# clearmatics/libff

Measured on AMD Instinct MI355X. Metric: G1 MSM throughput (scalar-muls/sec), higher is better.
Workload: dtype u32

## Files before the change

### libff_amd/build.py

```python
import concurrent.futures
import os
import shutil
import subprocess
import sys

HERE = os.path.dirname(os.path.abspath(__file__))
CSRC = os.path.join(HERE, "csrc")
OBJ = os.path.join(CSRC, "build")
INCLUDE = os.path.join(os.path.dirname(HERE), "include")
SO_PATH = os.path.join(HERE, "libamdmsm.so")

GROUPS = ["alt_bn128_g1", "alt_bn128_g2", "bls12_377_g1", "bls12_377_g2", "bw6_761_g1", "bw6_761_g2",
          "bls12_381_g1", "bls12_381_g2", "mnt4_g1", "mnt4_g2", "mnt6_g1"]
GROUP_FLAGS = {g: ["-DAMDMSM_HOT_INLINE=1", "-DAMDMSM_BENCH_BOTH=1"] for g in GROUPS}
GROUP_FLAGS["alt_bn128_g1"] = GROUP_FLAGS["alt_bn128_g1"] + ["-DAMDMSM_OVERLAP_OK=1"]
for _g in ("bls12_377_g2", "bls12_381_g2", "bw6_761_g1", "bw6_761_g2"):
    GROUP_FLAGS[_g] = GROUP_FLAGS[_g] + ["-DAMDMSM_ACC_WAVES=2"]
for _g in ("alt_bn128_g1", "bls12_377_g1", "bls12_381_g1"):
    GROUP_FLAGS[_g] = GROUP_FLAGS[_g] + ["-DAMDMSM_COLD_INLINE=1"]
for _g in ("bls12_377_g2", "bls12_381_g2", "alt_bn128_g2"):
    GROUP_FLAGS[_g] = GROUP_FLAGS[_g] + ["-DAMDMSM_ACC_SPLIT=1"]
GROUP_FLAGS["alt_bn128_g2"] = GROUP_FLAGS["alt_bn128_g2"] + ["-DAMDMSM_ACC_WAVES=3"]
for _g in ("bls12_377_g1", "bls12_381_g1"):
    GROUP_FLAGS[_g] = GROUP_FLAGS[_g] + ["-DAMDMSM_ACC_WAVES=3"]
for _g, _w in (("alt_bn128_g1", 3), ("bls12_377_g1", 2), ("bls12_381_g1", 2), ("bw6_761_g1", 2), ("bw6_761_g2", 2),
               ("alt_bn128_g2", 3), ("bls12_377_g2", 2), ("bls12_381_g2", 2)):
    GROUP_FLAGS[_g] = [f for f in GROUP_FLAGS[_g] if not f.startswith("-DAMDMSM_ACC_WAVES=")] + ["-DAMDMSM_ACC_RR=1", f"-DAMDMSM_ACC_WAVES={_w}"]
for _g in ("mnt4_g1", "mnt6_g1"):
    GROUP_FLAGS[_g] = GROUP_FLAGS[_g] + ["-DAMDMSM_COLD_INLINE=1", "-DAMDMSM_ACC_WAVES=3"]
GROUP_FLAGS["mnt4_g2"] = GROUP_FLAGS["mnt4_g2"] + ["-DAMDMSM_ACC_WAVES=2"]
ARCH = "gfx950"
COMMON = ["-O3", "-std=c++17", "-fPIC", f"--offload-arch={ARCH}", "-I" + INCLUDE, "-I" + CSRC,
          "-Wno-unused-result"]
DEVICE_DEPS = ["msm_group.hip", "rr.cuh", "rr_chain.inc", "fp.cuh", "fp2.cuh", "fp2h.cuh", "ec.cuh", "wide.cuh", "wide28.cuh", "mac_chain.inc", "curve_params.h", "group_vtable.h", os.path.join(HERE, "build.py")]
HOST_DEPS = ["engine.cpp", "ffi.cpp", "engine_internal.h", "group_vtable.h", os.path.join(INCLUDE, "amdmsm.h"),
             os.path.join(INCLUDE, "libff_amd_ffi.h")]


def hipcc():
    exe = shutil.which("hipcc") or "/opt/rocm/bin/hipcc"
    if not os.path.exists(exe):
        raise RuntimeError("hipcc not found: the amdmsm engine is HIP-only and cannot be built without ROCm")
    return exe


def _newer(target, deps):
    if not os.path.exists(target):
        return True
# ... 55 lines not shown
```

### libff_amd/csrc/engine.cpp

```cpp
#include "../../include/amdmsm.h"
#include "engine_internal.h"
#include "group_vtable.h"

#include <hip/hip_runtime.h>

#include <fcntl.h>
#include <sys/stat.h>
#include <unistd.h>

#include <algorithm>
#include <cmath>
#include <cstdio>
#include <cstdlib>
#include <cstring>
#include <mutex>
#include <string>
#include <thread>
#include <vector>

using namespace amdmsm;

constexpr int MAX_SLOTS = 4;
constexpr int MAX_GROUPS = 4;
struct ws_slot {
// ... 251 lines not shown
    p.off_plast = off;
    off = align_up(off + Wt * p.T * zz_bytes, 256);
    p.off_cont = off;
    off = align_up(off + Wt * p.T * 4, 256);
    p.G = G_req > 0 ? std::min(std::min(G_req, MAX_GROUPS), p.W) : 1;
    p.off_queue = off;
    p.queue_stride = align_up(fixup_queue_words((size_t)((p.W + p.G - 1) / p.G) * (size_t)batch * p.T) * 4, 256);
    off = off + p.queue_stride * p.G;
    p.off_partial = off;
    off = align_up(off + (size_t)MAX_GROUPS * xyz_bytes, 256);
    p.off_coarse = off;
    off = align_up(off + Wt * 1025 * 4, 256);
    p.off_big = off;
    p.big_stride = p.c <= 22 ? align_up(std::max(sort_geometry(n, p.c, p.W).big_words, big_words_min) * 4, 256) : 256;
    off += p.big_stride * (size_t)batch;
    p.off_cursor = off;
    off = align_up(off + Wt * 1024 * 4, 256);
    p.off_tmp_payload = off;
    off = align_up(off + Wt * p.list_stride * 4, 256);
    p.off_tmp_key = off;
    off = align_up(off + Wt * p.list_stride * 4, 256);
    p.off_endo = off;
    p.endo_stride = glv ? align_up((n / 2) * (size_t)vt->el_words * 2 * 4, 256) : 0;
    off += p.endo_stride * (size_t)batch;
    {
        static const int rc_env = getenv("AMDMSM_ROWCOL") ? atoi(getenv("AMDMSM_ROWCOL")) : 1;
        static const int rc_min_c = getenv("AMDMSM_ROWCOL_MIN_C") ? atoi(getenv("AMDMSM_ROWCOL_MIN_C")) : 10;
        static const int qr_env = getenv("AMDMSM_ROWCOL_QROW") ? atoi(getenv("AMDMSM_ROWCOL_QROW")) : 0;
        static const int qc_env = getenv("AMDMSM_ROWCOL_QCOL") ? atoi(getenv("AMDMSM_ROWCOL_QCOL")) : 0;
        p.rowcol = rc_env != 0 && p.c >= rc_min_c;
        const int h = p.c / 2;
        const size_t C = (size_t)1 << h, R = p.B >> h;
        const bool one_wave = vt->fq_words >= 24 || vt->el_words > vt->fq_words;
        const size_t lane_budget = one_wave ? 70000 : 140000;
        uint32_t q = 4;
        while (q < 64 && Wt * p.B * red_lanes * 2 / q > lane_budget) q <<= 1;
        p.q_row = qr_env > 0 ? (uint32_t)qr_env : q;
        p.q_col = qc_env > 0 ? (uint32_t)qc_env : q;
        p.rc_points = R + 1 + C;
        p.off_rc = off;
        off = align_up(off + Wt * p.rc_points * xyz_bytes, 256);
        p.off_planes = off;
        off = align_up(off + Wt * p.c * xyz_bytes, 256);
        p.off_winsum = off;
        off = align_up(off + Wt * xyz_bytes, 256);
    }
    p.total = off;
    return AMDMSM_OK;
}

int ensure_ws(amdmsm_ctx *ctx, ws_slot &sl, size_t bytes) {
    if (sl.ws_bytes >= bytes) return AMDMSM_OK;
    if (sl.ws) {
        HIP_TRY(ctx, hipDeviceSynchronize());
        HIP_TRY(ctx, hipFree(sl.ws));
        sl.ws = nullptr;
        sl.ws_bytes = 0;
    }
    const size_t want = bytes + bytes / 8;
    HIP_TRY(ctx, hipMalloc(&sl.ws, want));
    sl.ws_bytes = want;
    return AMDMSM_OK;
}

constexpr uint64_t TIMING_RING = 64;
void record(amdmsm_ctx *ctx, ws_slot &sl, int idx, hipStream_t st) {
    (void)sl;
// ... 2012 lines not shown
```

### libff_amd/csrc/group_vtable.h

```cpp
#pragma once
#include <hip/hip_runtime_api.h>
#include <stddef.h>
#include <stdint.h>
#include <stdlib.h>

namespace amdmsm {

enum out_form : int {
    OUT_JACOBIAN = 0,
    OUT_LIBFF = 1,
    OUT_AFFINE = 2,
};

struct sort_geom {
    int hb;
    int fb;
    uint32_t chunk_cap;
    uint32_t big_thresh;
    uint32_t big_cap;
    size_t big_words;
};
inline sort_geom sort_geometry(size_t n, int c, int W) {
    sort_geom g;
    static const int hb_env = getenv("AMDMSM_SORT_HB") ? atoi(getenv("AMDMSM_SORT_HB")) : 0;
    g.hb = c / 2 < 10 ? c / 2 : 10;
    if (c == 16 && n >= ((size_t)3 << 18) && n < ((size_t)3 << 19)) g.hb = 7;
    if (hb_env > 0) g.hb = hb_env;
    if (g.hb > c - 1) g.hb = c - 1;
    if (g.hb < 1) g.hb = 1;
    if (c - 1 - g.hb > 11) g.hb = c - 1 - 11;
    g.fb = c - 1 - g.hb;
    g.chunk_cap = 1024;
    static const uint32_t chunk_max = getenv("AMDMSM_SORT_CHUNK_MAX") ? (uint32_t)atoi(getenv("AMDMSM_SORT_CHUNK_MAX")) : 16384u;
    while (g.chunk_cap < chunk_max && g.chunk_cap < 2 * (n >> g.hb)) g.chunk_cap <<= 1;
    g.big_thresh = 16 * g.chunk_cap;
    g.big_cap = (uint32_t)((size_t)W * n / g.big_thresh + 1);
    g.big_words = 4 + (size_t)g.big_cap * 4 + ((size_t)g.big_cap << g.fb);
    return g;
}

#ifdef __HIPCC__
#define AMDMSM_HD __host__ __device__
#else
#define AMDMSM_HD
#endif
AMDMSM_HD inline size_t fixup_queue_cap_long(size_t lanes) { return lanes / 32 + 2; }
AMDMSM_HD inline size_t fixup_queue_cap_mid(size_t lanes) { return lanes / 3 + 2; }
inline size_t fixup_queue_words(size_t lanes) { return 2 + 2 * (fixup_queue_cap_long(lanes) + fixup_queue_cap_mid(lanes)); }

struct group_vtable {
    int curve, group;
    int fr_words;
    int el_words;
    int fq_words;
    int fr_bits;
    int projective;
    int reduce_fold;
    int bucket_words;
    const uint32_t* fr_one_mont;
    int glv_bound_log2_x1000;
    int prime_order;
    const uint32_t* glv_lambda;
    void (*endo_points)(hipStream_t, const uint32_t* bases_affine, size_t n, uint32_t* out);
    void (*glv_digits)(hipStream_t, const uint32_t* scalars, size_t n, int mont, int c, int W, int32_t* out);

    void (*import_bases)(hipStream_t, const uint32_t* src, size_t stride_words, int form_special,
                         size_t n, uint32_t* dst_affine);
    void (*precompute_table)(hipStream_t, const uint32_t* bases_affine, size_t n, int c, int D, uint32_t* tmp,
                             uint32_t* table);
    void (*count)(hipStream_t, const uint32_t* scalars, size_t n, int mont, int c, int W, uint32_t* counts);
    void (*scatter)(hipStream_t, const uint32_t* scalars, size_t n, int mont, int c, int W, uint32_t* cursor,
                    uint32_t* lists, size_t list_stride);
    void (*scalar_stats)(hipStream_t, const uint32_t* scalars, size_t n, int mont, uint32_t* stats);
    void (*sort)(hipStream_t, const uint32_t* scalars, size_t n, int mont, int c, int W, uint32_t* coarse,
                 uint32_t* cursor, int32_t* digits, uint32_t* tmp_payload, uint32_t* tmp_key, uint32_t* ends,
                 uint32_t* lists, size_t stride, uint32_t* big, int mode, hipEvent_t after_coarse);
    void (*accumulate)(hipStream_t, const uint32_t* ends, const uint32_t* lists, size_t list_stride,
                       const uint32_t* bases_affine, uint32_t* buckets, uint32_t* part_first, uint32_t* part_last,
                       uint32_t* cont_bucket, int W, uint32_t B, uint32_t S, uint32_t T, const uint32_t* endo_points,
                       size_t n_real, int overlap);
    size_t (*accumulate_resident_lanes)(int overlap);
    int accumulate_overlap_ok;
    void (*accumulate_fixup)(hipStream_t, const uint32_t* ends, uint32_t* buckets, uint32_t* part_first,
                             const uint32_t* part_last, const uint32_t* cont_bucket, uint32_t* queue, int W,
                             uint32_t B, uint32_t S, uint32_t T);
    void (*reduce_segments)(hipStream_t, const uint32_t* buckets, int W, uint32_t B, uint32_t L, uint32_t* out);
    void (*sum_butterfly)(hipStream_t, const uint32_t* in, int W, uint32_t M, uint32_t* out);
    void (*sum_block)(hipStream_t, const uint32_t* in, int W, uint32_t M, uint32_t* out);
    void (*reduce_rowcol)(hipStream_t, const uint32_t* buckets, int W, uint32_t B, int c, uint32_t q_row, uint32_t q_col,
                          uint32_t* rc, uint32_t* planes, uint32_t* out);
    void (*horner)(hipStream_t, const uint32_t* window_sums, int W, int c, int form, const uint32_t* init,
                   uint32_t* out);
    void (*horner_batch)(hipStream_t, const uint32_t* window_sums, int k, int W, int c, int form, uint32_t* const* outs);
    void (*sum_points)(hipStream_t, const uint32_t* pts, int k, int form, uint32_t* out);
    void (*gen_bases_seq)(hipStream_t, unsigned long long first, size_t n, uint32_t* dst_affine);
    void (*export_affine)(hipStream_t, const uint32_t* src_affine, size_t n, uint32_t* dst_xyz);

    void (*ffi_decode_points)(hipStream_t, const uint32_t* src_be, size_t n, uint32_t* dst_affine, uint32_t* status);
    void (*ffi_decode_scalars)(hipStream_t, const uint32_t* src_be, size_t n, uint32_t* dst_plain, uint32_t* status);
    void (*ffi_encode_point)(hipStream_t, const uint32_t* src_xyz_affine, uint32_t* dst_be);

    void (*disk_decode)(hipStream_t, const uint32_t* src, size_t n, uint32_t* dst_affine);
    void (*disk_decode_compressed)(hipStream_t, const uint32_t* src, size_t n, uint32_t* dst_affine, uint32_t* status);
    void (*fixed_base_exp)(hipStream_t, const uint32_t* g_xyz, int scalar_size, int window, const uint32_t* scalars,
                           size_t n, int mont, const uint32_t* coeff, int form, uint32_t* gouter, uint32_t* table,
                           uint32_t* table_aff, int build_table, uint32_t* out);

    void (*field_op)(hipStream_t, int op, const uint32_t* a, const uint32_t* b, uint32_t* out, size_t n);
    void (*group_op)(hipStream_t, int op, const uint32_t* a, const uint32_t* b, uint32_t* out, size_t n, int form);
    void (*digits)(hipStream_t, const uint32_t* scalars, size_t n, int mont, int c, int W, int32_t* out);
    void (*mul_bench)(hipStream_t, uint32_t* inout, size_t nthreads, int iters, int inline_variant);
    void (*madd_bench)(hipStream_t, const uint32_t* pts_affine, uint32_t* out_xyz, size_t nthreads, int iters,
                       int inline_variant);

    int has_endomorphism;
    int coeff_a_nonzero;

    void (*sort_sel)(hipStream_t, const uint32_t* shared, size_t shared_n, const uint32_t* index, size_t offset,
                     uint32_t* flag, size_t n, int mont, int c, int W, uint32_t* coarse, uint32_t* cursor, int32_t* digits,
                     uint32_t* tmp_payload, uint32_t* tmp_key, uint32_t* ends, uint32_t* lists, size_t stride, uint32_t* big,
                     int mode);
    void (*gather_scalars)(hipStream_t, const uint32_t* shared, size_t shared_n, const uint32_t* index, size_t offset,
                           uint32_t* flag, size_t n, uint32_t* out);
// ... 16 lines not shown
```

### libff_amd/csrc/msm_group.hip

```cpp
#include "curve_params.h"
#include "ec.cuh"
#include "fp2h.cuh"
#include "group_vtable.h"
#include "wide.cuh"
#include "wide28.cuh"
#include "rr.cuh"

#include <algorithm>
#include <cstdio>
#include <vector>
#include <type_traits>

#ifndef AMDMSM_GROUP
#error "compile with -DAMDMSM_GROUP=<group traits> -DAMDMSM_VT=<vtable getter name>"
#endif

namespace amdmsm {
template <bool I>
struct ec_coeff_a<Fp<AMDMSM_GROUP::fq, I>> {
    static constexpr int value = AMDMSM_GROUP::DEG == 1 ? AMDMSM_GROUP::COEFF_A : 0;
};
template <int NR, bool I>
struct ec_coeff_a<Fp2<AMDMSM_GROUP::fq, NR, I>> {
    static constexpr int value = AMDMSM_GROUP::DEG == 2 ? AMDMSM_GROUP::COEFF_A : 0;
};
namespace {

using GP = AMDMSM_GROUP;
using FQ = typename GP::fq;
using FR = typename GP::fr;
static_assert(GP::COEFF_A == 0 || (!GP::HAS_ENDO && GP::SUBGROUP_CHECK == 0 && GP::LIBFF_PROJECTIVE),
              "a != 0 is implemented for the MNT groups: no endomorphism, no subgroup test, projective records");
#if AMDMSM_ACC_RR || AMDMSM_ACC_SPLIT
static_assert(GP::COEFF_A == 0, "the reduced-radix and lane-pair accumulation loops are written for a = 0");
#endif

#ifndef AMDMSM_HOT_INLINE
#define AMDMSM_HOT_INLINE 0
#endif
#ifndef AMDMSM_BENCH_BOTH
#define AMDMSM_BENCH_BOTH 0
#endif
#ifndef AMDMSM_ACC_LAZY
#define AMDMSM_ACC_LAZY 1
#endif
#ifndef AMDMSM_ACC_WAVES
#define AMDMSM_ACC_WAVES 1
#endif
#ifndef AMDMSM_OVERLAP_OK
#define AMDMSM_OVERLAP_OK 0
#endif
#ifndef AMDMSM_TAIL_WAVES
#define AMDMSM_TAIL_WAVES 1
#endif
template <int DEG, bool I> struct coord_sel;
template <bool I> struct coord_sel<1, I> { using type = Fp<FQ, I>; };
template <bool I> struct coord_sel<2, I> { using type = Fp2<FQ, GP::NR_SMALL == 0 ? -1 : GP::NR_SMALL, I>; };
#ifndef AMDMSM_COLD_INLINE
#define AMDMSM_COLD_INLINE 0
#endif
using E = typename coord_sel<GP::DEG, (AMDMSM_COLD_INLINE != 0)>::type;
using EH = typename coord_sel<GP::DEG, (AMDMSM_HOT_INLINE != 0)>::type;
using EI = typename coord_sel<GP::DEG, true>::type;
#ifndef AMDMSM_ACC_SPLIT
#define AMDMSM_ACC_SPLIT 0
#endif
template <int DEG> struct split_sel { using type = EH; static constexpr int LANES = 1; };
#if AMDMSM_ACC_SPLIT
template <> struct split_sel<2> { using type = Fp2H<FQ, (GP::NR_SMALL == 0 ? -1 : GP::NR_SMALL)>; static constexpr int LANES = 2; };
#endif
using EA = typename split_sel<GP::DEG>::type;
constexpr int ACC_LANES = split_sel<GP::DEG>::LANES;
using ER = typename std::conditional<(ACC_LANES == 2), EA, E>::type;
constexpr int RED_LANES = ACC_LANES;
constexpr uint32_t RED_FOLD = 64u / RED_LANES;
#if AMDMSM_ACC_RR
static_assert(GP::DEG == 1 || AMDMSM_ACC_SPLIT, "reduced-radix Fq2 accumulation works on lane pairs");
template <int DEG> struct rr_el_sel { using type = Rr<FQ>; };
template <> struct rr_el_sel<2> { using type = Rr2H<FQ, (GP::NR_SMALL == 0 ? -1 : GP::NR_SMALL)>; };
using ERR = typename rr_el_sel<GP::DEG>::type;
#endif

constexpr int EW = FQ::N * GP::DEG;
constexpr int AFFW = 2 * EW;
constexpr int XYZW = 3 * EW;
constexpr int ZZW = 4 * EW;
#ifndef AMDMSM_ACC_RR
// ... 608 lines not shown
                                                        uint32_t perchunk_words, uint32_t* __restrict__ big,
                                                        uint32_t* __restrict__ ends, uint32_t* __restrict__ lists) {
    extern __shared__ __attribute__((aligned(16))) uint32_t smem[];
    __shared__ uint32_t tmp[NT / 64 + 1];
    const uint32_t nbin = 1u << hb;
    const int fb = c - 1 - hb;
    const uint32_t nfine = 1u << fb, fmask = nfine - 1u;
    uint32_t* fstart = smem;
    uint32_t* chist = fstart + nfine;
    uint32_t* cstart = chist + nfine;
    uint32_t* ccur = cstart + nfine;
    uint32_t* st_payload = ccur + nfine;
    unsigned short* st_fine = reinterpret_cast<unsigned short*>(st_payload + chunk_cap);
    const uint32_t bin = blockIdx.x, w = blockIdx.y;
    const uint32_t* cs = coarse + (size_t)w * (nbin + 1);
    const uint32_t b0 = cs[bin], m = cs[bin + 1] - b0;
    const sort_key_t* key = tmp_key + (size_t)w * stride + b0;
    const uint32_t* pay = tmp_payload + (size_t)w * stride + b0;
    uint32_t* out = lists + (size_t)w * stride + b0;
    uint32_t* e = ends + (((size_t)w << (c - 1)) + ((size_t)bin << fb));
    if (m > big_thresh) {
        for (uint32_t j = threadIdx.x; j < nfine; j += NT) e[j] = 0;
        if (threadIdx.x == 0) {
            const uint32_t tiles = (m + SORT_TILE - 1) / SORT_TILE;
            const uint32_t slot = atomicAdd(&big[0], 1u);
            uint32_t* rec = big + 4 + 4 * (size_t)slot;
            rec[0] = w;
            rec[1] = bin;
            rec[2] = atomicAdd(&big[1], tiles);
            rec[3] = tiles;
        }
        return;
    }
    if (m <= chunk_cap) {
        constexpr int PER = 16;
        uint32_t fk[PER], rk[PER];
        for (uint32_t j = threadIdx.x; j < nfine; j += NT) chist[j] = 0;
        __syncthreads();
#pragma unroll
        for (int q = 0; q < PER; ++q) {
            const uint32_t k = threadIdx.x + (uint32_t)q * NT;
            fk[q] = k < m ? (uint32_t)(key[k] & fmask) : 0u;
            rk[q] = k < m ? atomicAdd(&chist[fk[q]], 1u) : 0u;
        }
        __syncthreads();
        block_exclusive_scan<NT>(chist, fstart, nfine, tmp);
        for (uint32_t j = threadIdx.x; j < nfine; j += NT) e[j] = b0 + fstart[j] + chist[j];
#pragma unroll
        for (int q = 0; q < PER; ++q) {
            const uint32_t k = threadIdx.x + (uint32_t)q * NT;
            if (k < m) st_payload[fstart[fk[q]] + rk[q]] = pay[k];
        }
        __syncthreads();
        for (uint32_t k = threadIdx.x; k < m; k += NT) out[k] = st_payload[k];
        return;
    }
    const uint32_t nch = (m + chunk_cap - 1) / chunk_cap;
    const bool single = false;
    uint32_t* ch = reinterpret_cast<uint32_t*>(st_fine + chunk_cap);
    const bool split_hist = !single && (size_t)nch * nfine <= perchunk_words;
    if (split_hist) {
        int sh = 0;
        while ((1u << sh) < chunk_cap) ++sh;
        for (uint32_t j = threadIdx.x; j < nch * nfine; j += NT) ch[j] = 0;
        __syncthreads();
        for (uint32_t k = threadIdx.x; k < m; k += NT) atomicAdd(&ch[(k >> sh) * nfine + (key[k] & fmask)], 1u);
        __syncthreads();
        for (uint32_t j = threadIdx.x; j < nfine; j += NT) {
            uint32_t t = 0;
            for (uint32_t q = 0; q < nch; ++q) t += ch[q * nfine + j];
            chist[j] = t;
        }
    } else {
        for (uint32_t j = threadIdx.x; j < nfine; j += NT) chist[j] = 0;
        __syncthreads();
        for (uint32_t k = threadIdx.x; k < m; k += NT) atomicAdd(&chist[key[k] & fmask], 1u);
    }
    __syncthreads();
    block_exclusive_scan<NT>(chist, fstart, nfine, tmp);
    for (uint32_t j = threadIdx.x; j < nfine; j += NT) e[j] = b0 + fstart[j] + chist[j];
    __syncthreads();
    uint32_t cidx = 0;
    for (uint32_t c0 = 0; c0 < m; c0 += chunk_cap, ++cidx) {
        const uint32_t cm = (m - c0 < chunk_cap) ? m - c0 : chunk_cap;
        const uint32_t* hist_c = split_hist ? ch + cidx * nfine : chist;
        if (single) {
            for (uint32_t j = threadIdx.x; j < nfine; j += NT) cstart[j] = ccur[j] = fstart[j];
        } else {
            if (!split_hist) {
                for (uint32_t j = threadIdx.x; j < nfine; j += NT) chist[j] = 0;
                __syncthreads();
                for (uint32_t k = threadIdx.x; k < cm; k += NT) atomicAdd(&chist[key[c0 + k] & fmask], 1u);
                __syncthreads();
            }
            block_exclusive_scan<NT>(hist_c, cstart, nfine, tmp);
            for (uint32_t j = threadIdx.x; j < nfine; j += NT) ccur[j] = cstart[j];
        }
        __syncthreads();
        for (uint32_t k = threadIdx.x; k < cm; k += NT) {
            const uint32_t f = key[c0 + k] & fmask;
            const uint32_t r = atomicAdd(&ccur[f], 1u);
            st_payload[r] = pay[c0 + k];
            st_fine[r] = (unsigned short)f;
        }
        __syncthreads();
        for (uint32_t k = threadIdx.x; k < cm; k += NT) {
            const uint32_t f = st_fine[k];
            out[fstart[f] + (k - cstart[f])] = st_payload[k];
        }
        __syncthreads();
        for (uint32_t j = threadIdx.x; j < nfine; j += NT) fstart[j] += hist_c[j];
        __syncthreads();
    }
}

struct big_tile {
    uint32_t rec, w, bin, k0, cm;
};
AMDMSM_DEV bool big_find_tile(const uint32_t* __restrict__ big, const uint32_t* __restrict__ coarse, uint32_t nbin,
                              uint32_t tile, uint32_t* sh, big_tile& bt, uint32_t& b0) {
    const uint32_t nbig = big[0];
    __syncthreads();
    for (uint32_t r = threadIdx.x; r < nbig; r += SORT_TPB) {
        const uint32_t* rec = big + 4 + 4 * (size_t)r;
        if (tile >= rec[2] && tile < rec[2] + rec[3]) sh[0] = r;
    }
    __syncthreads();
    bt.rec = sh[0];
    const uint32_t* rec = big + 4 + 4 * (size_t)bt.rec;
    bt.w = rec[0];
// ... 247 lines not shown
        for (int j = 0; j < 4; ++j) {
            const int i = 4 * k + j;
            int32_t& dst = i < RRL ? re_limb(p.x, i) : (i < 2 * RRL ? re_limb(p.y, i - RRL) : (i < 3 * RRL ? re_limb(p.zz, i - 2 * RRL) : re_limb(p.zzz, i - 3 * RRL)));
            dst = (int32_t)w[j];
            if (i >= 2 * RRL && i < 3 * RRL) any |= w[j];
        }
    }
    inf = re_all<ERR>(any == 0);
    const bool rho = re_limb(p.zz, 0) < 0;
    if (rho) re_limb(p.zz, 0) &= 0x7fffffff;
    else xyzz_rec_to_rho(p);
}
AMDMSM_DEV void rec_sum_store(uint32_t* q, const rec_sum& s) {
    uint4* q4 = reinterpret_cast<uint4*>(q + (GP::DEG == 2 && (threadIdx.x & 1u) ? 4 * RRL : 0));
    uint32_t w[4 * RRL];
    const uint32_t keep = s.inf ? 0u : 0xffffffffu;
#pragma unroll
    for (int i = 0; i < RRL; ++i) {
        w[i] = (uint32_t)re_limb(s.a.x, i) & keep;
        w[RRL + i] = (uint32_t)re_limb(s.a.y, i) & keep;
        w[2 * RRL + i] = (uint32_t)re_limb(s.a.zz, i) & keep;
        w[3 * RRL + i] = (uint32_t)re_limb(s.a.zzz, i) & keep;
    }
    w[2 * RRL] |= 0x80000000u & keep;
#pragma unroll
    for (int i = 0; i < RRL; ++i) q4[i] = make_uint4(w[4 * i], w[4 * i + 1], w[4 * i + 2], w[4 * i + 3]);
}
AMDMSM_DEV void rec_sum_add(rec_sum& s, const uint32_t* q) {
    XyzzRr<ERR> b;
    bool b_inf;
    rec_load_rho(b, b_inf, q);
    xyzz_add_rho(s.a, s.inf, b, b_inf);
}
AMDMSM_DEV void rec_sum_fold(rec_sum& s, uint32_t G) {
    for (uint32_t off = 1; off < G; off <<= 1) {
        XyzzRr<ERR> o;
        const int m = (int)(off * RED_LANES);
#pragma unroll
        for (int i = 0; i < RRL; ++i) {
            re_limb(o.x, i) = __shfl_xor(re_limb(s.a.x, i), m, 64);
            re_limb(o.y, i) = __shfl_xor(re_limb(s.a.y, i), m, 64);
            re_limb(o.zz, i) = __shfl_xor(re_limb(s.a.zz, i), m, 64);
            re_limb(o.zzz, i) = __shfl_xor(re_limb(s.a.zzz, i), m, 64);
        }
        const bool o_inf = __shfl_xor(s.inf ? 1 : 0, m, 64) != 0;
        xyzz_add_rho(s.a, s.inf, o, o_inf);
    }
}
AMDMSM_DEV void rec_sum_get(Xyzz<ER>& out, const rec_sum& s) {
    if (s.inf) {
        xyzz_set_inf(out);
        return;
    }
    rr_export_component<FQ, 0>(lane_words(out.x), re_comp(s.a.x));
    rr_export_component<FQ, 0>(lane_words(out.y), re_comp(s.a.y));
    rr_export_component<FQ, 0>(lane_words(out.zz), re_comp(s.a.zz));
    rr_export_component<FQ, 0>(lane_words(out.zzz), re_comp(s.a.zzz));
}
#else
struct rec_sum {
    Xyzz<ER> a;
};
AMDMSM_DEV void rec_sum_init(rec_sum& s) { xyzz_set_inf(s.a); }
AMDMSM_DEV void rec_sum_add(rec_sum& s, const uint32_t* q) {
    Xyzz<ER> x;
    load_xyzz_rec(x, q);
    xyzz_add(s.a, s.a, x);
}
AMDMSM_DEV void rec_sum_get(Xyzz<ER>& out, const rec_sum& s) { out = s.a; }
AMDMSM_DEV void rec_sum_store(uint32_t* q, const rec_sum& s) { store_xyzz_rec(q, s.a); }
AMDMSM_DEV void wave_group_sum_r(Jac<ER>& p, uint32_t G);
AMDMSM_DEV void rec_sum_fold(rec_sum& s, uint32_t G) {
    Jac<ER> j;
    xyzz_to_jac(j, s.a);
    wave_group_sum_r(j, G);
    jac_to_xyzz(s.a, j);
}
#endif

AMDMSM_DEV uint32_t bucket_of_entry(const uint32_t* __restrict__ e, uint32_t B, uint32_t k) {
    uint32_t l = 0, r = B - 1;
    while (l < r) {
        const uint32_t m = (l + r) >> 1;
        if (e[m] > k) r = m; else l = m + 1;
    }
    return l;
}

__global__ void __launch_bounds__(TPB, AMDMSM_ACC_WAVES) k_accumulate(const uint32_t* __restrict__ ends, const uint32_t* __restrict__ lists,
                                                    size_t list_stride, const uint32_t* __restrict__ bases,
                                                    uint32_t* __restrict__ buckets, uint32_t* __restrict__ part_first,
                                                    uint32_t* __restrict__ part_last, uint32_t* __restrict__ cont_bucket,
                                                    int W, uint32_t B, uint32_t S, uint32_t T,
                                                    const uint32_t* __restrict__ endo_pts, uint32_t n_real, int sync_waves
#ifdef AMDMSM_ACC_TRACE
                                                    , unsigned long long* __restrict__ trace
#endif
                                                    ) {
#ifdef AMDMSM_ACC_TRACE
    const unsigned long long t_start = __builtin_amdgcn_s_memrealtime();
    struct trace_end {
// ... 394 lines not shown
            o[EW + env.j] = Y1;
            o[2 * EW + env.j] = Z1;
        }
    }
}
__global__ void __launch_bounds__(SUMW_THREADS) k_sum_block_wide(const uint32_t* __restrict__ in, int W, uint32_t M,
                                                                 uint32_t* __restrict__ out) {
    __shared__ uint32_t buf[2][SUMW_SLOTS * XYZW];
    __builtin_amdgcn_s_setprio(3);
    const size_t w = blockIdx.x;
    const uint32_t i = threadIdx.x / RED_LANES, wave = threadIdx.x >> 6;
    constexpr uint32_t NWAVES = SUMW_THREADS / 64;
    Jac<ER> p;
    if (i < M) load_jac(p, in + (w * M + i) * XYZW); else jac_set_inf(p);
    wave_group_sum_r(p, 4);
    if ((i & 3u) == 0) store_jac(buf[0] + (size_t)(i >> 2) * XYZW, p);
    __syncthreads();
    const WideEnv<FQ> env = wide_env<FQ>();
    uint32_t K = (M + 3) / 4;
    int cur = 0;
    while (K > 1) {
        const uint32_t pairs = K / 2;
        for (uint32_t q = wave; q < pairs; q += NWAVES) {
            const uint32_t* a = buf[cur] + (size_t)(2 * q) * XYZW;
            sum_wide_add(env, a, a + XYZW, buf[cur ^ 1] + (size_t)q * XYZW);
        }
        __syncthreads();
        cur ^= 1;
        K = pairs;
    }
    for (uint32_t t = threadIdx.x; t < (uint32_t)XYZW; t += SUMW_THREADS) out[w * XYZW + t] = buf[cur][t];
}

__global__ void __launch_bounds__(64, AMDMSM_TAIL_WAVES) k_bucket_sums(const uint32_t* __restrict__ buckets, int W, uint32_t B, int h,
                                                    uint32_t q_row, uint32_t q_col, uint32_t row_blocks,
                                                    uint32_t* __restrict__ out) {
    __builtin_amdgcn_s_setprio(3);
    const bool col = blockIdx.x >= row_blocks;
    const size_t t = ((size_t)(blockIdx.x - (col ? row_blocks : 0u)) * 64 + threadIdx.x) / RED_LANES;
    const uint32_t C = 1u << h, R = B >> h;
    const uint32_t q = col ? q_col : q_row, len = col ? R : C;
    const uint32_t g = len / q;
    const uint32_t nout = col ? C : R + 1;
    const size_t per_w = (size_t)nout * g;
    const size_t w = t / per_w;
    const uint32_t rem = (uint32_t)(t % per_w), o = rem / g, j = rem % g;
    const bool valid = w < (size_t)W;
    rec_sum sum;
    rec_sum_init(sum);
    if (valid) {
        const uint32_t* bk = buckets + w * (size_t)B * ZZS;
        for (uint32_t i = 0; i < q; ++i) {
            const uint32_t idx = j * q + i;
            const uint64_t b1 = col ? (uint64_t)idx * C + o : (uint64_t)o * C + idx;
            if (b1 >= 1 && b1 <= B) rec_sum_add(sum, bk + (size_t)(b1 - 1) * ZZS);
        }
    }
    rec_sum_fold(sum, g);
    Xyzz<ER> xa;
    rec_sum_get(xa, sum);
    Jac<ER> p;
    xyzz_to_jac(p, xa);
    if (valid && j == 0) store_jac(out + (w * (size_t)(R + 1 + C) + (col ? R + 1 + o : o)) * XYZW, p);
}

__global__ void __launch_bounds__(256) k_plane_sums(const uint32_t* __restrict__ rc, int W, int c, int h,
                                                     uint32_t* __restrict__ planes) {
    __shared__ uint32_t part[4 * XYZW];
    __builtin_amdgcn_s_setprio(3);
    const uint32_t w = blockIdx.x / (uint32_t)c, k = blockIdx.x % (uint32_t)c;
    const uint32_t C = 1u << h, R = (1u << (c - 1)) >> h, NP = R + 1 + C;
    const bool from_cols = k < (uint32_t)h;
    const uint32_t* src = rc + ((size_t)w * NP + (from_cols ? R + 1 : 0)) * XYZW;
    const uint32_t bit = from_cols ? k : k - (uint32_t)h;
    const bool top = k == (uint32_t)c - 1;
    const uint32_t M = top ? 1u : (from_cols ? C : R) / 2;
    const uint32_t nlanes = blockDim.x / RED_LANES, i0 = threadIdx.x / RED_LANES;
    const uint32_t lane = threadIdx.x & 63u, wave = threadIdx.x >> 6, nw = blockDim.x >> 6;
    Jac<ER> p, x;
    jac_set_inf(p);
    for (uint32_t i = i0; i < M; i += nlanes) {
        const uint32_t idx = top ? R : (((i >> bit) << (bit + 1)) | (1u << bit) | (i & ((1u << bit) - 1u)));
        load_jac(x, src + (size_t)idx * XYZW);
        jac_add(p, p, x);
    }
    wave_group_sum_r(p, RED_FOLD);
    if (lane < (uint32_t)RED_LANES) store_jac(part + wave * XYZW, p);
    __syncthreads();
    if (wave != 0) return;
    const uint32_t jw = lane / RED_LANES;
    if (jw < nw) load_jac(p, part + jw * XYZW); else jac_set_inf(p);
    uint32_t G = 1;
    while (G < nw) G <<= 1;
    wave_group_sum_r(p, G);
    if (lane < (uint32_t)RED_LANES) store_jac(planes + ((size_t)w * c + k) * XYZW, p);
}
// ... 1102 lines not shown
    };
    static const size_t lanes = query(0);
    static const size_t lanes_overlap = (AMDMSM_OVERLAP_OK && ACC_OVERLAP_LDS) ? query(ACC_OVERLAP_LDS) : lanes;
    return overlap ? lanes_overlap : lanes;
}
void l_accumulate_fixup(hipStream_t st, const uint32_t* ends, uint32_t* buckets, uint32_t* part_first,
                        const uint32_t* part_last, const uint32_t* cont_bucket, uint32_t* queue, int W, uint32_t B,
                        uint32_t S, uint32_t T) {
    const unsigned fix_blocks = blocks_for((size_t)W * T * RED_LANES, 64);
    const unsigned compact_blocks = T / FIX_BLOCK >= 2 ? (unsigned)(W * (T / FIX_BLOCK - 1)) : 0u;
    hipLaunchKernelGGL(k_accumulate_fixup, dim3(fix_blocks + compact_blocks), dim3(64), 0, st, ends, part_first,
                       part_last, cont_bucket, buckets, queue, W, B, S, T, fix_blocks);
    const size_t lanes = (size_t)W * T;
    const size_t cap_mid = fixup_queue_cap_mid(lanes) / (RED_FOLD / MID_G) + 1, cap_long = fixup_queue_cap_long(lanes);
    const unsigned mid_blocks = (unsigned)(cap_mid < 8192 ? cap_mid : 8192), long_blocks = (unsigned)(cap_long < 2048 ? cap_long : 2048);
    hipLaunchKernelGGL(k_accumulate_fixup_queue, dim3(mid_blocks + long_blocks), dim3(64), 0, st, ends,
                       part_first, part_last, cont_bucket, buckets, queue, mid_blocks, lanes, B, S, T);
}
void l_reduce_segments(hipStream_t st, const uint32_t* buckets, int W, uint32_t B, uint32_t L, uint32_t* out) {
    hipLaunchKernelGGL(k_reduce_segments, dim3(blocks_for((size_t)W * (B / L) * RED_LANES, 64)), dim3(64), 0, st, buckets, W, B,
                       L, out);
}
void l_sum_butterfly(hipStream_t st, const uint32_t* in, int W, uint32_t M, uint32_t* out) {
    hipLaunchKernelGGL(k_sum_butterfly, dim3(blocks_for((size_t)W * M * RED_LANES, 64)), dim3(64), 0, st, in, W, M, out);
}
void l_sum_block(hipStream_t st, const uint32_t* in, int W, uint32_t M, uint32_t* out) {
    if (M >= 8 && M * RED_LANES <= (uint32_t)SUMW_THREADS && (M & (M - 1)) == 0) {
        hipLaunchKernelGGL(k_sum_block_wide, dim3(W), dim3(SUMW_THREADS), 0, st, in, W, M, out);
        return;
    }
    const unsigned threads = (unsigned)((M * RED_LANES + 63) / 64 * 64);
    hipLaunchKernelGGL(k_sum_block, dim3(W), dim3(threads), 0, st, in, W, M, out);
}
void l_reduce_rowcol(hipStream_t st, const uint32_t* buckets, int W, uint32_t B, int c, uint32_t q_row, uint32_t q_col,
                     uint32_t* rc, uint32_t* planes, uint32_t* out) {
    const int h = c / 2;
    const uint32_t C = 1u << h, R = B >> h;
    auto fit = [](uint32_t len, uint32_t q) {
        if (q < 1) q = 1;
        while (q & (q - 1)) q &= q - 1;
        if (q > len) q = len;
        while (len / q > RED_FOLD) q <<= 1;
        return q;
    };
    q_row = fit(C, q_row);
    q_col = fit(R, q_col);
    const size_t row_lanes = (size_t)W * (R + 1) * (C / q_row) * RED_LANES, col_lanes = (size_t)W * C * (R / q_col) * RED_LANES;
    const unsigned row_blocks = blocks_for(row_lanes, 64), col_blocks = blocks_for(col_lanes, 64);
    hipLaunchKernelGGL(k_bucket_sums, dim3(row_blocks + col_blocks), dim3(64), 0, st, buckets, W, B, h, q_row, q_col, row_blocks, rc);
    const uint32_t maxm = (C > R ? C : R) / 2;
    static const bool wide_planes = !(getenv("AMDMSM_PLANES_WIDE") && atoi(getenv("AMDMSM_PLANES_WIDE")) == 0);
    if (maxm >= 8 && wide_planes) {
        hipLaunchKernelGGL(k_plane_sums_wide, dim3((unsigned)(W * c)), dim3(SUMW_THREADS), 0, st, rc, W, c, h, planes);
    } else {
        unsigned threads = (unsigned)((maxm * RED_LANES + 63) / 64 * 64);
        threads = threads < 64 ? 64 : (threads > 256 ? 256 : threads);
        hipLaunchKernelGGL(k_plane_sums, dim3((unsigned)(W * c)), dim3(threads), 0, st, rc, W, c, h, planes);
    }
    hipLaunchKernelGGL(k_window_horner, dim3((unsigned)W), dim3((unsigned)(64 * ((c + 3) / 4))), 0, st, planes, c, out);
}
void l_horner(hipStream_t st, const uint32_t* window_sums, int W, int c, int form, const uint32_t* init, uint32_t* out) {
    hipLaunchKernelGGL(k_horner, dim3(1), dim3(64), 0, st, window_sums, W, c, form, init, out);
}
void l_horner_batch(hipStream_t st, const uint32_t* window_sums, int k, int W, int c, int form, uint32_t* const* outs) {
    horner_outs o = {};
    for (int j = 0; j < k && j < 8; ++j) o.p[j] = outs[j];
    hipLaunchKernelGGL(k_horner_batch, dim3((unsigned)k), dim3(64), 0, st, window_sums, W, c, form, o);
}
void l_sum_points(hipStream_t st, const uint32_t* pts, int k, int form, uint32_t* out) {
    hipLaunchKernelGGL(k_sum_points, dim3(1), dim3(64), 0, st, pts, k, form, out);
}
void l_gen_bases_seq(hipStream_t st, unsigned long long first, size_t n, uint32_t* dst) {
    if (!n) return;
    hipLaunchKernelGGL(k_gen_bases_seq, dim3(blocks_for(n)), dim3(TPB), 0, st, first, n, dst);
}
void l_export_affine(hipStream_t st, const uint32_t* src, size_t n, uint32_t* dst) {
    if (!n) return;
    hipLaunchKernelGGL(k_export_affine, dim3(blocks_for(n)), dim3(TPB), 0, st, src, n, dst);
}
void l_ffi_decode_points(hipStream_t st, const uint32_t* src, size_t n, uint32_t* dst, uint32_t* status) {
// ... 62 lines not shown
}
void l_digits(hipStream_t st, const uint32_t* scalars, size_t n, int mont, int c, int W, int32_t* out) {
    if (!n) return;
    hipLaunchKernelGGL(k_digits, dim3(blocks_for(n)), dim3(TPB), 0, st, scalars, n, mont, c, W, out);
}
void l_mul_bench(hipStream_t st, uint32_t* inout, size_t nthreads, int iters, int inline_variant) {
    if (!nthreads) return;
#if AMDMSM_BENCH_BOTH
    if (inline_variant) {
        hipLaunchKernelGGL(k_mul_bench<true>, dim3(blocks_for(nthreads)), dim3(TPB), 0, st, inout, nthreads, iters);
        return;
    }
#endif
    hipLaunchKernelGGL(k_mul_bench<false>, dim3(blocks_for(nthreads)), dim3(TPB), 0, st, inout, nthreads, iters);
}
void l_madd_bench(hipStream_t st, const uint32_t* pts, uint32_t* out, size_t nthreads, int iters, int inline_variant) {
    if (!nthreads) return;
    if (inline_variant == 2) {
        hipLaunchKernelGGL(k_xyzz_madd_bench<EH>, dim3(blocks_for(nthreads)), dim3(TPB), 0, st, pts, out, nthreads, iters);
        return;
    }
#if AMDMSM_BENCH_BOTH
    if (inline_variant) {
        hipLaunchKernelGGL(k_madd_bench<EI>, dim3(blocks_for(nthreads)), dim3(TPB), 0, st, pts, out, nthreads, iters);
        return;
    }
#endif
    hipLaunchKernelGGL(k_madd_bench<E>, dim3(blocks_for(nthreads)), dim3(TPB), 0, st, pts, out, nthreads, iters);
}

const group_vtable g_vt = {
    GP::CURVE, GP::GROUP, FRW, EW, FQ::N, FR::BITS, GP::LIBFF_PROJECTIVE ? 1 : 0, (int)RED_FOLD, ZZS, FR::R,
    GLV::BOUND_LOG2_X1000, GP::SUBGROUP_CHECK == 0 ? 1 : 0, GLV::LAMBDA, l_endo_points, l_glv_digits,
    l_import_bases, l_precompute_table, l_count, l_scatter, l_scalar_stats, l_sort, l_accumulate, l_accumulate_resident_lanes, (AMDMSM_OVERLAP_OK && ACC_OVERLAP_LDS) ? 1 : 0, l_accumulate_fixup, l_reduce_segments, l_sum_butterfly, l_sum_block, l_reduce_rowcol, l_horner, l_horner_batch, l_sum_points,
    l_gen_bases_seq, l_export_affine, l_ffi_decode_points, l_ffi_decode_scalars, l_ffi_encode_point, l_disk_decode, l_disk_decode_compressed, l_fixed_base_exp, l_field_op, l_group_op, l_digits, l_mul_bench, l_madd_bench,
    GP::HAS_ENDO ? 1 : 0, GP::COEFF_A != 0 ? 1 : 0, l_sort_sel, l_gather_scalars,
};

}

const group_vtable* AMDMSM_VT() { return &g_vt; }

}
```

Measured before the change: 616.1 million.

## Size row/col bucket-sum split from occupancy; drop alt_bn128 G1 overlap mode

Removes the overlap-mode flag for alt_bn128_g1 and adds a static_assert tying overlap mode to tail register caps. The rowcol q-selection lane budget for multi-wave groups now comes from measured resident occupancy of k_bucket_sums instead of a fixed constant. The row pass skips a separate work item for the top bucket by copying it directly, which trims launched lanes. The sort kernel's single-chunk path also gains a size guard and dead code is removed. Dropping overlap mode may lose the accumulate/LDS overlap on the benchmarked G1 group.

```diff
diff --git a/libff_amd/build.py b/libff_amd/build.py
--- a/libff_amd/build.py
+++ b/libff_amd/build.py
@@ -13,7 +13,6 @@
 GROUPS = ["alt_bn128_g1", "alt_bn128_g2", "bls12_377_g1", "bls12_377_g2", "bw6_761_g1", "bw6_761_g2",
           "bls12_381_g1", "bls12_381_g2", "mnt4_g1", "mnt4_g2", "mnt6_g1"]
 GROUP_FLAGS = {g: ["-DAMDMSM_HOT_INLINE=1", "-DAMDMSM_BENCH_BOTH=1"] for g in GROUPS}
-GROUP_FLAGS["alt_bn128_g1"] = GROUP_FLAGS["alt_bn128_g1"] + ["-DAMDMSM_OVERLAP_OK=1"]
 for _g in ("bls12_377_g2", "bls12_381_g2", "bw6_761_g1", "bw6_761_g2"):
     GROUP_FLAGS[_g] = GROUP_FLAGS[_g] + ["-DAMDMSM_ACC_WAVES=2"]
 for _g in ("alt_bn128_g1", "bls12_377_g1", "bls12_381_g1"):
diff --git a/libff_amd/csrc/engine.cpp b/libff_amd/csrc/engine.cpp
--- a/libff_amd/csrc/engine.cpp
+++ b/libff_amd/csrc/engine.cpp
@@ -307,7 +307,8 @@
         const int h = p.c / 2;
         const size_t C = (size_t)1 << h, R = p.B >> h;
         const bool one_wave = vt->fq_words >= 24 || vt->el_words > vt->fq_words;
-        const size_t lane_budget = one_wave ? 70000 : 140000;
+        const size_t resident = vt->bucket_sums_resident_lanes() * red_lanes;
+        const size_t lane_budget = one_wave ? 70000 : (resident ? resident : 140000);
         uint32_t q = 4;
         while (q < 64 && Wt * p.B * red_lanes * 2 / q > lane_budget) q <<= 1;
         p.q_row = qr_env > 0 ? (uint32_t)qr_env : q;
diff --git a/libff_amd/csrc/group_vtable.h b/libff_amd/csrc/group_vtable.h
--- a/libff_amd/csrc/group_vtable.h
+++ b/libff_amd/csrc/group_vtable.h
@@ -31,7 +31,10 @@
     if (c - 1 - g.hb > 11) g.hb = c - 1 - 11;
     g.fb = c - 1 - g.hb;
     g.chunk_cap = 1024;
-    static const uint32_t chunk_max = getenv("AMDMSM_SORT_CHUNK_MAX") ? (uint32_t)atoi(getenv("AMDMSM_SORT_CHUNK_MAX")) : 16384u;
+    static const uint32_t chunk_max = [] {
+        const long v = getenv("AMDMSM_SORT_CHUNK_MAX") ? atol(getenv("AMDMSM_SORT_CHUNK_MAX")) : 16384;
+        return (uint32_t)(v < 1024 ? 1024 : (v > 16384 ? 16384 : v));
+    }();
     while (g.chunk_cap < chunk_max && g.chunk_cap < 2 * (n >> g.hb)) g.chunk_cap <<= 1;
     g.big_thresh = 16 * g.chunk_cap;
     g.big_cap = (uint32_t)((size_t)W * n / g.big_thresh + 1);
@@ -89,6 +92,7 @@
     void (*sum_block)(hipStream_t, const uint32_t* in, int W, uint32_t M, uint32_t* out);
     void (*reduce_rowcol)(hipStream_t, const uint32_t* buckets, int W, uint32_t B, int c, uint32_t q_row, uint32_t q_col,
                           uint32_t* rc, uint32_t* planes, uint32_t* out);
+    size_t (*bucket_sums_resident_lanes)();
     void (*horner)(hipStream_t, const uint32_t* window_sums, int W, int c, int form, const uint32_t* init,
                    uint32_t* out);
     void (*horner_batch)(hipStream_t, const uint32_t* window_sums, int k, int W, int c, int form, uint32_t* const* outs);
diff --git a/libff_amd/csrc/msm_group.hip b/libff_amd/csrc/msm_group.hip
--- a/libff_amd/csrc/msm_group.hip
+++ b/libff_amd/csrc/msm_group.hip
@@ -53,6 +53,7 @@
 #ifndef AMDMSM_TAIL_WAVES
 #define AMDMSM_TAIL_WAVES 1
 #endif
+static_assert(!AMDMSM_OVERLAP_OK || AMDMSM_TAIL_WAVES >= 4, "overlap mode needs tail kernels capped at 128 registers (AMDMSM_TAIL_WAVES=4)");
 template <int DEG, bool I> struct coord_sel;
 template <bool I> struct coord_sel<1, I> { using type = Fp<FQ, I>; };
 template <bool I> struct coord_sel<2, I> { using type = Fp2<FQ, GP::NR_SMALL == 0 ? -1 : GP::NR_SMALL, I>; };
@@ -727,8 +728,8 @@
         }
         return;
     }
-    if (m <= chunk_cap) {
-        constexpr int PER = 16;
+    constexpr int PER = 16;
+    if (m <= chunk_cap && m <= (uint32_t)PER * NT) {
         uint32_t fk[PER], rk[PER];
         for (uint32_t j = threadIdx.x; j < nfine; j += NT) chist[j] = 0;
         __syncthreads();
@@ -751,9 +752,8 @@
         return;
     }
     const uint32_t nch = (m + chunk_cap - 1) / chunk_cap;
-    const bool single = false;
     uint32_t* ch = reinterpret_cast<uint32_t*>(st_fine + chunk_cap);
-    const bool split_hist = !single && (size_t)nch * nfine <= perchunk_words;
+    const bool split_hist = (size_t)nch * nfine <= perchunk_words;
     if (split_hist) {
         int sh = 0;
         while ((1u << sh) < chunk_cap) ++sh;
@@ -779,18 +779,14 @@
     for (uint32_t c0 = 0; c0 < m; c0 += chunk_cap, ++cidx) {
         const uint32_t cm = (m - c0 < chunk_cap) ? m - c0 : chunk_cap;
         const uint32_t* hist_c = split_hist ? ch + cidx * nfine : chist;
-        if (single) {
-            for (uint32_t j = threadIdx.x; j < nfine; j += NT) cstart[j] = ccur[j] = fstart[j];
-        } else {
-            if (!split_hist) {
-                for (uint32_t j = threadIdx.x; j < nfine; j += NT) chist[j] = 0;
-                __syncthreads();
-                for (uint32_t k = threadIdx.x; k < cm; k += NT) atomicAdd(&chist[key[c0 + k] & fmask], 1u);
-                __syncthreads();
-            }
-            block_exclusive_scan<NT>(hist_c, cstart, nfine, tmp);
-            for (uint32_t j = threadIdx.x; j < nfine; j += NT) ccur[j] = cstart[j];
-        }
+        if (!split_hist) {
+            for (uint32_t j = threadIdx.x; j < nfine; j += NT) chist[j] = 0;
+            __syncthreads();
+            for (uint32_t k = threadIdx.x; k < cm; k += NT) atomicAdd(&chist[key[c0 + k] & fmask], 1u);
+            __syncthreads();
+        }
+        block_exclusive_scan<NT>(hist_c, cstart, nfine, tmp);
+        for (uint32_t j = threadIdx.x; j < nfine; j += NT) ccur[j] = cstart[j];
         __syncthreads();
         for (uint32_t k = threadIdx.x; k < cm; k += NT) {
             const uint32_t f = key[c0 + k] & fmask;
@@ -1104,6 +1100,7 @@
     rec_load_rho(b, b_inf, q);
     xyzz_add_rho(s.a, s.inf, b, b_inf);
 }
+AMDMSM_DEV void rec_sum_set(rec_sum& s, const uint32_t* q) { rec_load_rho(s.a, s.inf, q); }
 AMDMSM_DEV void rec_sum_fold(rec_sum& s, uint32_t G) {
     for (uint32_t off = 1; off < G; off <<= 1) {
         XyzzRr<ERR> o;
@@ -1139,6 +1136,7 @@
     load_xyzz_rec(x, q);
     xyzz_add(s.a, s.a, x);
 }
+AMDMSM_DEV void rec_sum_set(rec_sum& s, const uint32_t* q) { load_xyzz_rec(s.a, q); }
 AMDMSM_DEV void rec_sum_get(Xyzz<ER>& out, const rec_sum& s) { out = s.a; }
 AMDMSM_DEV void rec_sum_store(uint32_t* q, const rec_sum& s) { store_xyzz_rec(q, s.a); }
 AMDMSM_DEV void wave_group_sum_r(Jac<ER>& p, uint32_t G);
@@ -1599,6 +1597,7 @@
     for (uint32_t t = threadIdx.x; t < (uint32_t)XYZW; t += SUMW_THREADS) out[w * XYZW + t] = buf[cur][t];
 }
 
+__host__ __device__ inline bool row_copies_top(uint32_t g) { return g > 1; }
 __global__ void __launch_bounds__(64, AMDMSM_TAIL_WAVES) k_bucket_sums(const uint32_t* __restrict__ buckets, int W, uint32_t B, int h,
                                                     uint32_t q_row, uint32_t q_col, uint32_t row_blocks,
                                                     uint32_t* __restrict__ out) {
@@ -1608,15 +1607,16 @@
     const uint32_t C = 1u << h, R = B >> h;
     const uint32_t q = col ? q_col : q_row, len = col ? R : C;
     const uint32_t g = len / q;
-    const uint32_t nout = col ? C : R + 1;
+    const bool copy_top = !col && row_copies_top(g);
+    const uint32_t nout = col ? C : R + (copy_top ? 0u : 1u);
     const size_t per_w = (size_t)nout * g;
     const size_t w = t / per_w;
     const uint32_t rem = (uint32_t)(t % per_w), o = rem / g, j = rem % g;
     const bool valid = w < (size_t)W;
     rec_sum sum;
     rec_sum_init(sum);
+    const uint32_t* bk = buckets + (valid ? w : 0) * (size_t)B * ZZS;
     if (valid) {
-        const uint32_t* bk = buckets + w * (size_t)B * ZZS;
         for (uint32_t i = 0; i < q; ++i) {
             const uint32_t idx = j * q + i;
             const uint64_t b1 = col ? (uint64_t)idx * C + o : (uint64_t)o * C + idx;
@@ -1624,11 +1624,13 @@
         }
     }
     rec_sum_fold(sum, g);
+    const bool top = valid && copy_top && o == R - 1 && j == g - 1;
+    if (top) rec_sum_set(sum, bk + (size_t)(B - 1) * ZZS);
     Xyzz<ER> xa;
     rec_sum_get(xa, sum);
     Jac<ER> p;
     xyzz_to_jac(p, xa);
-    if (valid && j == 0) store_jac(out + (w * (size_t)(R + 1 + C) + (col ? R + 1 + o : o)) * XYZW, p);
+    if (valid && (j == 0 || top)) store_jac(out + (w * (size_t)(R + 1 + C) + (col ? R + 1 + o : (top ? R : o))) * XYZW, p);
 }
 
 __global__ void __launch_bounds__(256) k_plane_sums(const uint32_t* __restrict__ rc, int W, int c, int h,
@@ -2797,6 +2799,18 @@
     const unsigned threads = (unsigned)((M * RED_LANES + 63) / 64 * 64);
     hipLaunchKernelGGL(k_sum_block, dim3(W), dim3(threads), 0, st, in, W, M, out);
 }
+size_t l_bucket_sums_resident_lanes() {
+    static const size_t lanes = [] {
+        int dev = 0, cus = 0, blocks = 0;
+        if (hipGetDevice(&dev) != hipSuccess || hipDeviceGetAttribute(&cus, hipDeviceAttributeMultiprocessorCount, dev) != hipSuccess ||
+            hipOccupancyMaxActiveBlocksPerMultiprocessor(&blocks, k_bucket_sums, 64, 0) != hipSuccess || cus <= 0 || blocks <= 0) {
+            (void)hipGetLastError();
+            return (size_t)0;
+        }
+        return (size_t)cus * (size_t)blocks * 64 / RED_LANES;
+    }();
+    return lanes;
+}
 void l_reduce_rowcol(hipStream_t st, const uint32_t* buckets, int W, uint32_t B, int c, uint32_t q_row, uint32_t q_col,
                      uint32_t* rc, uint32_t* planes, uint32_t* out) {
     const int h = c / 2;
@@ -2810,7 +2824,7 @@
     };
     q_row = fit(C, q_row);
     q_col = fit(R, q_col);
-    const size_t row_lanes = (size_t)W * (R + 1) * (C / q_row) * RED_LANES, col_lanes = (size_t)W * C * (R / q_col) * RED_LANES;
+    const size_t row_lanes = (size_t)W * (R + (row_copies_top(C / q_row) ? 0 : 1)) * (C / q_row) * RED_LANES, col_lanes = (size_t)W * C * (R / q_col) * RED_LANES;
     const unsigned row_blocks = blocks_for(row_lanes, 64), col_blocks = blocks_for(col_lanes, 64);
     hipLaunchKernelGGL(k_bucket_sums, dim3(row_blocks + col_blocks), dim3(64), 0, st, buckets, W, B, h, q_row, q_col, row_blocks, rc);
     const uint32_t maxm = (C > R ? C : R) / 2;
@@ -2939,7 +2953,7 @@
 const group_vtable g_vt = {
     GP::CURVE, GP::GROUP, FRW, EW, FQ::N, FR::BITS, GP::LIBFF_PROJECTIVE ? 1 : 0, (int)RED_FOLD, ZZS, FR::R,
     GLV::BOUND_LOG2_X1000, GP::SUBGROUP_CHECK == 0 ? 1 : 0, GLV::LAMBDA, l_endo_points, l_glv_digits,
-    l_import_bases, l_precompute_table, l_count, l_scatter, l_scalar_stats, l_sort, l_accumulate, l_accumulate_resident_lanes, (AMDMSM_OVERLAP_OK && ACC_OVERLAP_LDS) ? 1 : 0, l_accumulate_fixup, l_reduce_segments, l_sum_butterfly, l_sum_block, l_reduce_rowcol, l_horner, l_horner_batch, l_sum_points,
+    l_import_bases, l_precompute_table, l_count, l_scatter, l_scalar_stats, l_sort, l_accumulate, l_accumulate_resident_lanes, (AMDMSM_OVERLAP_OK && ACC_OVERLAP_LDS) ? 1 : 0, l_accumulate_fixup, l_reduce_segments, l_sum_butterfly, l_sum_block, l_reduce_rowcol, l_bucket_sums_resident_lanes, l_horner, l_horner_batch, l_sum_points,
     l_gen_bases_seq, l_export_affine, l_ffi_decode_points, l_ffi_decode_scalars, l_ffi_encode_point, l_disk_decode, l_disk_decode_compressed, l_fixed_base_exp, l_field_op, l_group_op, l_digits, l_mul_bench, l_madd_bench,
     GP::HAS_ENDO ? 1 : 0, GP::COEFF_A != 0 ? 1 : 0, l_sort_sel, l_gather_scalars,
 };
```

Result: no change. 615.1 million (median of 2 runs) (-0.2%).
